# genjax-dev/genjax

Measured on AMD Instinct MI355X. Metric: particles/sec (particle-steps/s), bootstrap SMC sweep, linear-Gaussian SSM T=100, higher is better.
Workload: dtype f32; 1 GPU; BASELINE config 2: linear-Gaussian state-space (T=100), bootstrap SMC, systematic resampling every step; particles_per_gpu=1000000, particles_total=1000000, T=100, resampler=systematic, graph=True, key=314159

## Files before the change

genjax_amd/csrc/gmx_block.h:

```cpp
#pragma once
#define GMX_CHAIN_PRIO 2
#define GMX_SETPRIO __builtin_amdgcn_s_setprio(GMX_CHAIN_PRIO);
#include "gmx_math.h"
#define GMX_RTC_TILE 1024
#define GMX_RTC_MAX_TILES 2048
#if !defined(__HIPCC_RTC__)
#include "gmx_sizes.h"
static_assert(GMX_TILE == GMX_RTC_TILE && GMX_MAX_TILES == GMX_RTC_MAX_TILES, "gmx_block.h restates gmx_sizes.h for hiprtc");
#else
#define GMX_TILE GMX_RTC_TILE
#define GMX_MAX_TILES GMX_RTC_MAX_TILES
#endif

#define GMX_BLOCK 256
#define GMX_WAVE 64

template <int CTRL, int ROWMASK>
__device__ __forceinline__ uint32_t gmx_dpp(uint32_t identity, uint32_t v) {
  return (uint32_t)__builtin_amdgcn_update_dpp((int)identity, (int)v, CTRL, ROWMASK, 0xf, false);
}
#define GMX_DPP_SCAN_STEPS(STEP) \
  STEP(0x111, 0xf) STEP(0x112, 0xf) STEP(0x114, 0xf) STEP(0x118, 0xf) STEP(0x142, 0xa) STEP(0x143, 0xc)

#define GMX_DPP_ASM_ENTER "s_nop 4\n\t"
#define GMX_DPP_ASM_STEPS(OP) \
  OP("row_shr:1 row_mask:0xf bank_mask:0xf") OP("row_shr:2 row_mask:0xf bank_mask:0xf") \
  OP("row_shr:4 row_mask:0xf bank_mask:0xf") OP("row_shr:8 row_mask:0xf bank_mask:0xf") \
  OP("row_bcast:15 row_mask:0xa bank_mask:0xf") OP("row_bcast:31 row_mask:0xc bank_mask:0xf")

__device__ __forceinline__ float wave_max_scan(float v) {
#define GMX_OP(CTRL) "s_nop 1\n\tv_max_f32_dpp %0, %0, %0 " CTRL "\n\t"
  asm(GMX_DPP_ASM_ENTER GMX_DPP_ASM_STEPS(GMX_OP) : "+v"(v));
#undef GMX_OP
  return v;
}
__device__ __forceinline__ float wave_max(float v) {
  return gmx_u2f((uint32_t)__builtin_amdgcn_readlane((int)gmx_f2u(wave_max_scan(v)), 63));
}
__device__ __forceinline__ float wave_sum(float v) {
#pragma unroll
  for (int m = 32; m >= 1; m >>= 1) v = v + __shfl_xor(v, m, GMX_WAVE);
  return v;
}
__device__ __forceinline__ float block_max(float v, float* lds4) {
  v = wave_max(v);
  int w = threadIdx.x >> 6;
  __syncthreads();
  if ((threadIdx.x & 63) == 0) lds4[w] = v;
  __syncthreads();
  float r = gmx_rmax(gmx_rmax(lds4[0], lds4[1]), gmx_rmax(lds4[2], lds4[3]));
  return r;
}
__device__ __forceinline__ float block_sum(float v, float* lds4) {
  v = wave_sum(v);
  int w = threadIdx.x >> 6;
  __syncthreads();
  if ((threadIdx.x & 63) == 0) lds4[w] = v;
  __syncthreads();
  float r = (lds4[0] + lds4[1]) + (lds4[2] + lds4[3]);
  return r;
}

__device__ __forceinline__ void gmx_red_max(float* red_out, float* lds4, uint32_t row, float x, bool active) {
  float m = block_max(active ? x : -gmx_inf(), lds4);
  if (threadIdx.x == 0 && red_out) red_out[row] = m;
}
__device__ __forceinline__ void gmx_red_lse(float* red_out, float* lds4, uint32_t row, uint32_t rows, float x,
                                            bool active) {
  float m = block_max(active ? x : -gmx_inf(), lds4);
  float e = active ? gmx_expf(x - m) : 0.0f;
  if (!(m > -gmx_inf())) e = 0.0f;
  float s = block_sum(e, lds4);
  if (threadIdx.x == 0 && red_out) {
    red_out[row] = m;
    red_out[(size_t)rows + row] = s;
  }
}

__device__ __forceinline__ uint64_t wave_scan_u64(uint64_t v) {
  uint32_t lo = (uint32_t)v, hi = (uint32_t)(v >> 32);
#define GMX_OP(CTRL) "s_nop 1\n\tv_add_co_u32_dpp %0, vcc, %0, %0 " CTRL "\n\tv_addc_co_u32_dpp %1, vcc, %1, %1, vcc " CTRL "\n\t"
  asm(GMX_DPP_ASM_ENTER GMX_DPP_ASM_STEPS(GMX_OP) : "+v"(lo), "+v"(hi) : : "vcc");
#undef GMX_OP
  return ((uint64_t)hi << 32) | lo;
}
__device__ __forceinline__ uint64_t wave_last_u64(uint64_t v) {
  uint32_t lo = (uint32_t)__builtin_amdgcn_readlane((int)(uint32_t)v, 63);
  uint32_t hi = (uint32_t)__builtin_amdgcn_readlane((int)(uint32_t)(v >> 32), 63);
  return ((uint64_t)hi << 32) | lo;
}
__device__ __forceinline__ uint64_t wave_sum_u64(uint64_t v) { return wave_last_u64(wave_scan_u64(v)); }
__device__ __forceinline__ uint32_t wave_shr1_u32(uint32_t v, uint32_t first) { return gmx_dpp<0x138, 0xf>(first, v); }
__device__ __forceinline__ uint64_t shfl_up_u64(uint64_t v, int d) {
  uint32_t lo = (uint32_t)v, hi = (uint32_t)(v >> 32);
  lo = __shfl_up(lo, d, GMX_WAVE);
  hi = __shfl_up(hi, d, GMX_WAVE);
  return ((uint64_t)hi << 32) | lo;
}

__device__ __forceinline__ uint64_t weight_fixed(float lw, float ref, float scale) {
  return gmx_exp_fixed(lw - ref, (int)(gmx_f2u(scale) >> 23) - 127);
}

#define GMX_TP_MAX_TILES GMX_MAX_TILES
#define GMX_TP_PER_MAX (GMX_TP_MAX_TILES / GMX_BLOCK)
__device__ __forceinline__ void gmx_tile_prefix_block(const float* tmax, const uint64_t* agg, int n_tiles,
                                                      uint64_t* pref, float* lds4, uint64_t* lds8) {
  const int tid = (int)threadIdx.x, lane = tid & 63, wave = tid >> 6;
  const int per = (n_tiles + GMX_BLOCK - 1) / GMX_BLOCK;
  uint64_t ta[GMX_TP_PER_MAX];
  float tm[GMX_TP_PER_MAX];
#pragma unroll
  for (int r = 0; r < GMX_TP_PER_MAX; ++r) {
    ta[r] = 0ull; tm[r] = -gmx_inf();
    if (r < per) {
      const int t = tid * per + r;
      const int tc = t < n_tiles ? t : n_tiles - 1;
      ta[r] = agg[tc];
      tm[r] = tmax[tc];
    }
  }
  float M = -gmx_inf();
#pragma unroll
  for (int r = 0; r < GMX_TP_PER_MAX; ++r) {
    if (r < per) {
      const bool ok = tid * per + r < n_tiles;
      ta[r] = ok ? ta[r] : 0ull;
      tm[r] = ok ? tm[r] : -gmx_inf();
      M = gmx_rmax(M, tm[r]);
    }
  }
  M = block_max(M, lds4);
  const int32_t K = gmx_tile_exp(M);
  uint64_t P[GMX_TP_PER_MAX];
  uint64_t run = 0;
#pragma unroll
  for (int r = 0; r < GMX_TP_PER_MAX; ++r) {
    P[r] = run;
    if (r < per) run += gmx_tile_scale(ta[r], gmx_tile_exp(tm[r]), K);
  }
  const uint64_t inc = wave_scan_u64(run);
  __syncthreads();
  if (lane == 63) lds8[wave] = inc;
  __syncthreads();
  uint64_t wave_off = 0, total = 0;
#pragma unroll
  for (int w = 0; w < 4; ++w) { const uint64_t v = lds8[w]; total += v; wave_off += (w < wave) ? v : 0ull; }
  const uint64_t base = wave_off + (inc - run);
#pragma unroll
  for (int r = 0; r < GMX_TP_PER_MAX; ++r) {
    if (r < per) {
      const int t = tid * per + r;
      if (t < n_tiles) pref[t] = base + P[r];
    }
  }
  if (tid == 0) {
    pref[n_tiles] = total;
    pref[n_tiles + 1] = (uint64_t)gmx_f2u(M) | ((uint64_t)(uint32_t)K << 32);
  }
}
```

genjax_amd/csrc/gmx_kernels.hip:

```cpp
#include <hip/hip_runtime.h>
#include <hip/hiprtc.h>
#include <stdio.h>
#include <stdlib.h>
#include <string.h>
#include <sys/stat.h>
#include <unistd.h>

#include <new>
#include <atomic>
#include <string>
#include <vector>

#include "gmx_block.h"
#include "gmx_vm.h"
#include "gmx_resample.h"
#include "gmx_peer.h"
#include "gmx_sorted.h"
#include "gmx_offspring.h"
#include "gmx_shard_fill.h"

#define GMX_HIP(call)                                                        \
  do {                                                                       \
    hipError_t _e = (call);                                                  \
    if (_e != hipSuccess) return gmx_fail("%s (hip error %lld)", hipGetErrorString(_e), (long long)_e); \
// ... 309 lines not shown
extern "C" int gmx_program_despecialize(gmx_program* p, const char* why) {
  if (!p) return gmx_fail("gmx_program_despecialize: null program%s");
  if (!p->jit_fn) return 0;
  (void)hipDeviceSynchronize();
  (void)hipModuleUnload(p->jit_module);
  p->jit_fn = nullptr; p->jit_module = nullptr; p->jit_code_hash = 0;
  ++g_jit_rejected;
  (void)gmx_fail("specialised kernel rejected, the interpreter takes over: %s", why ? why : "");
  return 0;
}
extern "C" uint64_t gmx_program_code_hash(const gmx_program* p) { return p && p->jit_fn ? p->jit_code_hash : 0ull; }
extern "C" int gmx_program_writes_tile_stats(const gmx_program* p) {
  return p && p->jit_fn && p->jit_pp == 4 && p->n_redmax == 1 && !p->uses_lse ? 1 : 0;
}

extern "C" int gmx_program_set_fuse_resample(gmx_program* p) {
  if (!p) return gmx_fail("gmx_program_set_fuse_resample: null program%s");
  if (p->jit_fn) return gmx_fail("gmx_program_set_fuse_resample: the program is already specialised%s");
  p->fuse_rs = true;
  return 0;
}
extern "C" int gmx_program_set_fuse_resample_loop(gmx_program* p) {
  if (!p) return gmx_fail("gmx_program_set_fuse_resample_loop: null program%s");
  if (p->jit_fn) return gmx_fail("gmx_program_set_fuse_resample_loop: the program is already specialised%s");
  p->fuse_rs = true;
  p->fuse_rs_loop = true;
  return 0;
}
static int64_t rs_loop_grid(const gmx_program* p, int64_t tiles) {
  int64_t g = p->jit_resident_blocks > 0 ? p->jit_resident_blocks : 256;
  if (g > 1024) g = 1024;

  return tiles < g ? tiles : g;
}
extern "C" int gmx_program_fuses_resample(const gmx_program* p) {
  return p && p->jit_fn && p->fuse_rs && p->jit_pp == 4 && p->uses_gather && p->jit_gathers_pre ? 1 : 0;
}
extern "C" int gmx_program_set_fuse_shard_step(gmx_program* p) {
  if (!p) return gmx_fail("gmx_program_set_fuse_shard_step: null program%s");
  if (p->jit_fn) return gmx_fail("gmx_program_set_fuse_shard_step: the program is already specialised%s");
  p->fuse_sh = true;
  return 0;
}
extern "C" int gmx_program_fuses_shard_step(const gmx_program* p) {
  return p && p->jit_fn && p->fuse_sh && p->jit_pp == 4 && p->uses_gather && p->jit_gathers_pre ? 1 : 0;
}
extern "C" int64_t gmx_program_resident_particles(const gmx_program* p) {
  if (!p || !p->jit_fn) return 0;
  if (p->fuse_rs_loop && p->jit_pp == 4 && p->jit_resident_blocks > 0)
    return rs_loop_grid(p, 1024) * 16 * (int64_t)GMX_BLOCK * 4;
  return p->jit_resident_blocks * (int64_t)GMX_BLOCK * (int64_t)p->jit_pp;
}

extern "C" int gmx_program_set_background(gmx_program* p, uint32_t lds_pad) {
  if (!p) return gmx_fail("gmx_program_set_background: null program%s");
  if (p->jit_fn) return gmx_fail("gmx_program_set_background: the program is already specialised%s");
  if (lds_pad > 160u * 1024u) return gmx_fail("gmx_program_set_background: lds_pad above the 160 KB of a CU%s");
  p->background = true;
  p->lds_pad = lds_pad;
  return 0;
}

static uint64_t fnv1a(uint64_t h, const char* s, size_t n) {
  for (size_t i = 0; i < n; ++i) { h ^= (unsigned char)s[i]; h *= 0x100000001b3ull; }
  return h;
}

static std::string jit_cache_dir() {
  const char* e = getenv("GENMI_JIT_CACHE");
  if (e && e[0] == '0' && e[1] == '\0') return "";
  if (e && e[0]) return e;
  const char* x = getenv("XDG_CACHE_HOME");
  if (x && x[0]) return std::string(x) + "/genjax_amd/jit";
  const char* h = getenv("HOME");
  if (h && h[0]) return std::string(h) + "/.cache/genjax_amd/jit";
  return "";
}

static void mkdirs(const std::string& d) {
  for (size_t i = 1; i <= d.size(); ++i)
    if (i == d.size() || d[i] == '/') (void)mkdir(d.substr(0, i).c_str(), 0755);
}

static std::string jit_cache_path(const std::string& src) {
  std::string dir = jit_cache_dir();
  if (dir.empty()) return "";
  uint64_t h = fnv1a(0xcbf29ce484222325ull, src.data(), src.size());
  for (int k = 0; k < GMX_EMBED_COUNT; ++k) h = fnv1a(h, gmx_embed_src[k], strlen(gmx_embed_src[k]));
  int major = 0, minor = 0;
  (void)hiprtcVersion(&major, &minor);
  char buf[64];
  snprintf(buf, sizeof(buf), "/%016llx_rtc%d.%d_abi%d_e2.co", (unsigned long long)h, major, minor, GMX_ABI_VERSION);
  return dir + buf;
}

static const char* jit_opt_level() {
  const char* e = getenv("GENMI_JIT_OPT");
  return (e && (!strcmp(e, "-O1") || !strcmp(e, "-O2") || !strcmp(e, "-O0"))) ? e : "-O3";
}

static bool jit_cache_read(const std::string& path, std::vector<char>& code) {
  if (strcmp(jit_opt_level(), "-O3") != 0) return false;
  if (path.empty()) return false;
  FILE* f = fopen(path.c_str(), "rb");
  if (!f) return false;
  bool ok = false;
  if (fseek(f, 0, SEEK_END) == 0) {
    long n = ftell(f);
    if (n > 0 && n < (64l << 20) && fseek(f, 0, SEEK_SET) == 0) {
      code.resize((size_t)n);
      ok = fread(code.data(), 1, (size_t)n, f) == (size_t)n;
    }
  }
  fclose(f);
  return ok;
}

static bool jit_under_profiler() {
  const char* e = getenv("ROCP_TOOL_LIBRARIES");
  if (e && e[0]) return true;
  e = getenv("LD_PRELOAD");
  return e && strstr(e, "rocprofiler") != nullptr;
}

static void jit_cache_write(const std::string& path, const std::vector<char>& code) {
  if (path.empty() || jit_under_profiler() || strcmp(jit_opt_level(), "-O3") != 0) return;
  if (const char* f_ = getenv("GENMI_JIT_FAULT")) { if (f_[0] == '1') return; }
  mkdirs(path.substr(0, path.rfind('/')));
  char tmp[32];
  snprintf(tmp, sizeof(tmp), ".tmp%ld", (long)getpid());
  std::string t = path + tmp;
  FILE* f = fopen(t.c_str(), "wb");
  if (!f) return;
  bool ok = fwrite(code.data(), 1, code.size(), f) == code.size();
  ok = (fclose(f) == 0) && ok;
  if (!ok || rename(t.c_str(), path.c_str()) != 0) (void)remove(t.c_str());
}

static int jit_compile(const std::string& src, std::vector<char>& code) {
  hiprtcProgram prog;
  const char* hdr_src[GMX_EMBED_COUNT];
  const char* hdr_name[GMX_EMBED_COUNT];
  for (int k = 0; k < GMX_EMBED_COUNT; ++k) { hdr_src[k] = gmx_embed_src[k]; hdr_name[k] = gmx_embed_name[k]; }
  hiprtcResult rc = hiprtcCreateProgram(&prog, src.c_str(), "gmx_jit_program.hip", GMX_EMBED_COUNT, hdr_src, hdr_name);
  if (rc != HIPRTC_SUCCESS) return gmx_fail("hiprtcCreateProgram: %s", hiprtcGetErrorString(rc));
  const char* opts[4] = {"--offload-arch=gfx950", jit_opt_level(), "-std=c++17", "-ffp-contract=off"};
  rc = hiprtcCompileProgram(prog, 4, opts);
  if (rc != HIPRTC_SUCCESS) {
    size_t ls = 0;
    hiprtcGetProgramLogSize(prog, &ls);
    std::string log(ls + 1, '\0');
    if (ls) hiprtcGetProgramLog(prog, &log[0]);
    hiprtcDestroyProgram(&prog);
    if (log.size() > 400) log.resize(400);
    return gmx_fail("hiprtcCompileProgram failed: %s", log.c_str());
  }
  size_t cs = 0;
  hiprtcGetCodeSize(prog, &cs);
  code.resize(cs);
  hiprtcGetCode(prog, code.data());
  hiprtcDestroyProgram(&prog);
  return 0;
}

static int jit_load(gmx_program* p, const std::vector<char>& code) {
  hipModule_t mod;
  GMX_HIP(hipModuleLoadData(&mod, code.data()));
  hipFunction_t fn;
  hipError_t e = hipModuleGetFunction(&fn, mod, p->background ? "gmx_jit_background_kernel" : "gmx_jit_kernel");
  if (e != hipSuccess) { (void)hipModuleUnload(mod); return gmx_fail("hipModuleGetFunction: %s", hipGetErrorString(e)); }
  p->jit_module = mod;
  p->jit_fn = fn;
  p->jit_pp = jit_pp_for(p);
  p->jit_code_hash = fnv1a(0xcbf29ce484222325ull, code.data(), code.size());
  if (p->lds_pad > 48 * 1024) {
    hipError_t ea = hipFuncSetAttribute((const void*)fn, hipFuncAttributeMaxDynamicSharedMemorySize, (int)p->lds_pad);
    if (ea != hipSuccess) { (void)hipGetLastError(); p->lds_pad = 48 * 1024; }
  }
  p->jit_resident_blocks = 0;
  int per_cu = 0, dev = 0, cus = 0;
  if (hipModuleOccupancyMaxActiveBlocksPerMultiprocessor(&per_cu, fn, GMX_BLOCK, (size_t)p->lds_pad) == hipSuccess &&
      hipGetDevice(&dev) == hipSuccess &&
      hipDeviceGetAttribute(&cus, hipDeviceAttributeMultiprocessorCount, dev) == hipSuccess)
    p->jit_resident_blocks = (int64_t)per_cu * (int64_t)cus;
  else
    (void)hipGetLastError();
  return 0;
}

extern "C" int gmx_program_specialize(gmx_program* p) {
  if (!p) return gmx_fail("gmx_program_specialize: null program%s");
  if (p->jit_fn) return 0;
  if (!jit_enabled()) return gmx_fail("gmx_program_specialize: disabled by GENMI_JIT=0%s");
  if (p->n_instr == 0 || p->n_instr > 8192) return gmx_fail("gmx_program_specialize: program size out of range%s");
  const std::string src = jit_source(p, &p->jit_gathers_pre);
  const std::string path = jit_cache_path(src);
  std::vector<char> code;
  if (jit_cache_read(path, code)) {
    if (jit_load(p, code) == 0) return 0;
    (void)hipGetLastError();
  }
  if (jit_compile(src, code)) return 1;
  if (jit_load(p, code)) return 1;
  jit_cache_write(path, code);
  return 0;
}

extern "C" size_t gmx_specialize_dryrun2(const uint32_t* blob, size_t n_words, int flags, char* log_out, size_t log_cap,
                                         char* code_out, size_t code_cap);
extern "C" size_t gmx_specialize_dryrun(const uint32_t* blob, size_t n_words, char* log_out, size_t log_cap,
                                        char* code_out, size_t code_cap) {
  return gmx_specialize_dryrun2(blob, n_words, 0, log_out, log_cap, code_out, code_cap);
}
extern "C" size_t gmx_specialize_dryrun2(const uint32_t* blob, size_t n_words, int flags, char* log_out, size_t log_cap,
                                         char* code_out, size_t code_cap) {
  gmx_program P;
  if (parse_program(blob, n_words, P)) { if (log_out && log_cap) snprintf(log_out, log_cap, "%s", gmx_err_); return 0; }
  P.fuse_rs = (flags & 1) != 0 || (flags & 8) != 0;
  P.fuse_rs_loop = (flags & 8) != 0;
  P.background = (flags & 2) != 0;
  P.fuse_sh = (flags & 4) != 0;
  const gmx_program* p = &P;
  std::string src = jit_source(p);
  hiprtcProgram prog;
  const char* hdr_src[GMX_EMBED_COUNT];
  const char* hdr_name[GMX_EMBED_COUNT];
  for (int k = 0; k < GMX_EMBED_COUNT; ++k) { hdr_src[k] = gmx_embed_src[k]; hdr_name[k] = gmx_embed_name[k]; }
  if (hiprtcCreateProgram(&prog, src.c_str(), "gmx_jit_program.hip", GMX_EMBED_COUNT, hdr_src, hdr_name) != HIPRTC_SUCCESS)
    return 0;
  const char* opts[] = {"--offload-arch=gfx950", "-O3", "-std=c++17", "-ffp-contract=off"};
  hiprtcResult rc = hiprtcCompileProgram(prog, 4, opts);
  size_t ls = 0;
  hiprtcGetProgramLogSize(prog, &ls);
  if (log_out && log_cap) {
    std::string log(ls + 1, '\0');
    if (ls) hiprtcGetProgramLog(prog, &log[0]);
    snprintf(log_out, log_cap, "%s", log.c_str());
  }
  size_t cs = 0;
  if (rc == HIPRTC_SUCCESS) {
    hiprtcGetCodeSize(prog, &cs);
    if (code_out && code_cap >= cs) hiprtcGetCode(prog, code_out);
  }
  hiprtcDestroyProgram(&prog);
  return cs;
}

extern "C" int64_t gmx_program_grid(const gmx_program* p, int64_t n) {
  int64_t per = GMX_BLOCK;
  if (p && p->jit_fn && !p->uses_lse) per = (int64_t)GMX_BLOCK * p->jit_pp;
  return (n + per - 1) / per;
}

static int peer_check(const char* who, const gmx_peer& P, int64_t n_per_rank);
extern "C" int gmx_program_run(const gmx_program* p, int64_t n, const gmx_run_args* args,
                               gmx_stream stream) {
  if (!p || !args) return gmx_fail("gmx_program_run: null argument%s");
  if (n < 0) return gmx_fail("gmx_program_run: negative n%s");
  if (n == 0) return 0;
  if (n > (int64_t)0x7fffffff * GMX_BLOCK) return gmx_fail("gmx_program_run: n too large%s");
  for (uint32_t s = 0; s < p->n_in; ++s)
    if (!args->in_d[s]) return gmx_fail("gmx_program_run: input slot %s%lld is null", "", s);
  for (uint32_t s = 0; s < p->n_out; ++s)
    if (!args->out_d[s]) return gmx_fail("gmx_program_run: output slot %s%lld is null", "", s);
  for (uint32_t s = 0; s < p->n_tab; ++s)
    if (!args->tab_d[s]) return gmx_fail("gmx_program_run: table slot %s%lld is null", "", s);
  if (p->uses_gather && !args->ancestors_d)
    return gmx_fail("gmx_program_run: program gathers but ancestors_d is null%s");
  const bool fused_rs = args->rs.lw_d != nullptr;
  if (fused_rs) {
    const gmx_resample_in& q = args->rs;
    if (!gmx_program_fuses_resample(p))
      return gmx_fail("gmx_program_run: rs is set but this program cannot resample in its own launch "
                      "(gmx_program_set_fuse_resample before specialising; 4 particles per thread; gathering)%s");
    if (!q.tile_max_d || !q.tile_agg_d || !q.max_out_d || !q.total_out_d || !q.status_d)
      return gmx_fail("gmx_program_run: rs has a null pointer%s");
    if ((uintptr_t)q.lw_d & 15) return gmx_fail("gmx_program_run: rs.lw_d must be 16-byte aligned%s");
    if ((!p->fuse_rs_loop && (n + RS_TILE - 1) / RS_TILE > 1024) || n > gmx_program_resident_particles(p) ||
        n > (int64_t)GMX_ANC_INDEX_MASK + 1)
      return gmx_fail("gmx_program_run: rs: every workgroup of the launch must be resident at once (n <= 2^20 and "
                      "n <= gmx_program_resident_particles(); a looped program — gmx_program_set_fuse_resample_loop — "
                      "walks up to 16 tiles per workgroup: n <= 2^24)%s");
    if (q.shift < 1 || q.shift > 62) return gmx_fail("gmx_program_run: rs.shift out of range%s");
    int need = 0;
    while (((int64_t)1 << need) < n) ++need;
    if (q.shift + need > 62) return gmx_fail("gmx_program_run: rs.shift too large for n (overflow)%s");
    if (q.tag < 1u || q.tag > GMX_ANC_TAG_MAX) return gmx_fail("gmx_program_run: rs.tag must be in [1, 255]%s");
    if (args->tile_agg_d == q.tile_agg_d || (const float*)args->red_out_d == q.tile_max_d)
      return gmx_fail("gmx_program_run: rs reads the tile statistics this launch writes (use two sets)%s");
    for (uint32_t s = 0; s < p->n_out; ++s)
      if ((const void*)args->out_d[s] == (const void*)q.lw_d)
        return gmx_fail("gmx_program_run: rs.lw_d is also an output of this launch (use two buffers)%s");
  }
  const bool fused_sh = args->sh.lw_d != nullptr;
  if (fused_sh) {
    const gmx_shard_in& q = args->sh;
    if (fused_rs) return gmx_fail("gmx_program_run: rs and sh are both set%s");
    if (!gmx_program_fuses_shard_step(p))
      return gmx_fail("gmx_program_run: sh is set but this program cannot route a sharded step in its own launch "
                      "(gmx_program_set_fuse_shard_step before specialising; 4 particles per thread; gathering)%s");
    if (!q.stats_own_d || !q.plan_d || !q.total_out_d || !q.max_out_d || !q.status_d)
      return gmx_fail("gmx_program_run: sh has a null pointer%s");
    if (((uintptr_t)q.lw_d & 15) || ((uintptr_t)q.stats_own_d & 7))
      return gmx_fail("gmx_program_run: sh.lw_d must be 16-byte and sh.stats_own_d 8-byte aligned%s");
    if (peer_check("gmx_program_run (sh)", q.peer, n)) return 1;
    if (q.peer.world > 8 || (int64_t)q.peer.world * q.peer.tiles > 4 * GMX_BLOCK)
      return gmx_fail("gmx_program_run: sh: world <= 8 and world * tiles <= 1024%s");
    if (n + (int64_t)q.peer.world * q.peer.capacity > (int64_t)GMX_ANC_INDEX_MASK + 1)
      return gmx_fail("gmx_program_run: sh: n + world * capacity must fit the 21-bit index of an ancestor word%s");
    if (n > gmx_program_resident_particles(p))
      return gmx_fail("gmx_program_run: sh: every workgroup of the launch must be resident at once "
                      "(n <= gmx_program_resident_particles())%s");
    if (q.shift < 1 || q.shift > 62) return gmx_fail("gmx_program_run: sh.shift out of range%s");
    if (q.tag < 1u || q.tag > GMX_ANC_TAG_MAX) return gmx_fail("gmx_program_run: sh.tag must be in [1, 255]%s");
// ... 2842 lines not shown
```

genjax_amd/csrc/gmx_offspring.h:

```cpp
#pragma once
#include "gmx_block.h"
#include "gmx_resample.h"
#include "gmx_sorted.h"

#define CDF_VEC_OT 4
#ifndef RS_THREADS
#define RS_THREADS 256
#endif
#define RS_TILE (RS_THREADS * CDF_VEC_OT)
#define RS_MAX_TILES GMX_MAX_TILES
static_assert(RS_TILE == GMX_TILE && RS_THREADS == GMX_BLOCK, "resampling tiles are the CDF's definition tiles");
static_assert(RS_MAX_TILES % GMX_BLOCK == 0, "tile table shape");

#define GMX_ANC_TAG_SHIFT 24
#define GMX_ANC_INDEX_MASK 0xffffffu
#define GMX_ANC_TAG_MAX 255u
__device__ __forceinline__ void gmx_store_u32x4_sc1(uint32_t* p, uint32_t a, uint32_t b, uint32_t c, uint32_t d) {
  typedef uint32_t v4 __attribute__((ext_vector_type(4)));
  v4 v; v.x = a; v.y = b; v.z = c; v.w = d;
  asm volatile("s_nop 1\n\tglobal_store_dwordx4 %0, %1, off sc1\n\ts_nop 1" :: "v"(p), "v"(v) : "memory");
}
__device__ __forceinline__ void gmx_store_u32_sc1(uint32_t* p, uint32_t a) {
  __hip_atomic_store(p, a, __ATOMIC_RELAXED, __HIP_MEMORY_SCOPE_AGENT);
}

typedef uint32_t rs_u32x4_a4 __attribute__((ext_vector_type(4), aligned(4)));
typedef uint32_t sorted_u32x2_a4 __attribute__((ext_vector_type(2), aligned(4)));
struct sorted_ctx {
  const uint32_t* slow; const uint32_t* guide; const uint64_t* toff;
  uint64_t stot, gmax; uint32_t sh, mask; double ratio;
};
__device__ __forceinline__ sorted_ctx sorted_ctx_of(const uint32_t* table, int64_t n, uint64_t total, uint64_t stot, uint32_t sh) {
  const gmx_sorted_layout L = gmx_sorted_layout_of(n);
  sorted_ctx X;
  X.slow = table; X.guide = table + L.off_guide;
  X.toff = reinterpret_cast<const uint64_t*>(table + L.off_toff);
  X.stot = stot;
  X.sh = sh;
  X.mask = (1u << X.sh) - 1u;
  X.gmax = X.stot >> X.sh;
  X.ratio = (double)X.stot / (double)(total ? total : 1ull);
  return X;
}
__device__ __forceinline__ int64_t sorted_below_exact(const sorted_ctx& X, uint64_t c, uint64_t total, int64_t j, int64_t n) {
  const u128 R = mul64(c, X.stot);
  j = j < 0 ? 0 : (j > n ? n : j);
  auto below = [&](int64_t k) {
    const uint64_t off = X.toff[k >> 10];
    const uint64_t S = off + (uint64_t)(uint32_t)(X.slow[k] - (uint32_t)off);
    return gt128(R, mul64(S, total));
  };
  while (j > 0 && !below(j - 1)) --j;
  while (j < n && below(j)) ++j;
  return j;
}

#define RS_TPB 1
#define GMX_KEEP_BRANCH asm volatile("")
#define RS_BLOCK (GMX_BLOCK * RS_TPB)
#define RS_WAVES (RS_BLOCK / GMX_WAVE)
static_assert(RS_MAX_TILES % RS_BLOCK == 0, "tile table shape");
#define RS_FILL_SLOTS 2048
template <int kind, int PER, bool TAGGED>
__device__ __forceinline__ void
gmx_offspring_tile_body(uint32_t k0, uint32_t k1, uint32_t u0_host, const float* __restrict__ lw,
                        const float* __restrict__ tmax, const uint64_t* __restrict__ agg, int64_t n, int n_tiles, float scale,
                        float* __restrict__ max_out, uint64_t* __restrict__ total_out, int32_t* __restrict__ anc,
                        const uint32_t* __restrict__ uslot, uint32_t tag,
                        int tile0 = -1, uint64_t a_prefix = 0ull, uint64_t a_total = 0ull, uint64_t a_mk = 0ull) {
  const int blk = tile0 >= 0 ? tile0 : (int)blockIdx.x;
  const uint32_t tagw = TAGGED ? (tag << GMX_ANC_TAG_SHIFT) : 0u;
  __shared__ uint64_t s_below[RS_WAVES], s_all[RS_WAVES], s_scan[RS_WAVES], s_g[RS_TPB];
  __shared__ float s_max[RS_WAVES];
  const int lane = threadIdx.x & 63, wave = threadIdx.x >> 6;
  const int grp = RS_TPB > 1 ? (int)(threadIdx.x >> 8) : 0, ltid = threadIdx.x & (GMX_BLOCK - 1);
  const int first_tile = blk * RS_TPB;
  const int my_tile = first_tile + grp;
  const bool tile_ok = my_tile < n_tiles;
  const int tile_c = tile_ok ? my_tile : n_tiles - 1;
  const int64_t i0 = (int64_t)tile_c * RS_TILE + (int64_t)ltid * CDF_VEC_OT;
  float x[CDF_VEC_OT];
  const bool full_tile = (int64_t)(tile_c + 1) * RS_TILE <= n;
  if (full_tile) {
    float4 v = *reinterpret_cast<const float4*>(lw + i0);
    x[0] = v.x; x[1] = v.y; x[2] = v.z; x[3] = v.w;
  } else {
#pragma unroll
    for (int c = 0; c < CDF_VEC_OT; ++c) {
      const int64_t ic = i0 + c < n ? i0 + c : n - 1;
      const float xv = lw[ic];
      x[c] = (i0 + c < n) ? xv : -gmx_inf();
    }
  }
  constexpr bool PREF = (PER == 0);
  constexpr int PERN = PREF ? 1 : PER;
  static_assert(PER >= 0 && PER * RS_BLOCK <= RS_MAX_TILES, "rows of the tile table per thread");
  static_assert(!PREF || RS_TPB == 1, "the prefix form works on one tile per block");
  uint64_t ta[PERN];
  float tm[PERN];
  uint64_t pf_prefix = 0, pf_total = 0, pf_mk = 0;
  if (PREF) {
    if (agg) { pf_prefix = agg[tile_c]; pf_total = agg[n_tiles]; pf_mk = agg[n_tiles + 1]; }
    else { pf_prefix = a_prefix; pf_total = a_total; pf_mk = a_mk; }
  } else {
#pragma unroll
    for (int r = 0; r < PERN; ++r) {
      ta[r] = 0ull; tm[r] = -gmx_inf();
      if (r * RS_BLOCK < n_tiles) {
        const int t = r * RS_BLOCK + (int)threadIdx.x;
        const int tc = t < n_tiles ? t : n_tiles - 1;
        ta[r] = agg[tc];
        tm[r] = tmax[tc];
      }
    }
  }
  const float tmax_mine = tmax[tile_c];
  uint64_t sx_stot = 0; uint32_t sx_sh = 0;
  if constexpr (kind == GMX_RESAMPLE_MULTINOMIAL_SORTED) {
    const gmx_sorted_layout L = gmx_sorted_layout_of(n);
    sx_stot = reinterpret_cast<const uint64_t*>(uslot + L.off_toff)[L.tiles];
    sx_sh = uslot[L.off_sh];
  }
  __builtin_amdgcn_sched_barrier(0);
  if (!PREF) {
#pragma unroll
    for (int r = 0; r < PERN; ++r) {
      if (r * RS_BLOCK < n_tiles && (r + 1) * RS_BLOCK > n_tiles) {
        GMX_KEEP_BRANCH;
        const int t = r * RS_BLOCK + (int)threadIdx.x;
        ta[r] = (t < n_tiles) ? ta[r] : 0ull;
        tm[r] = (t < n_tiles) ? tm[r] : -gmx_inf();
      }
    }
  }
  const int32_t k_b = gmx_tile_exp(tmax_mine);
  const float ref_b = gmx_tile_ref(k_b);
  float M = -gmx_inf();
  if (PREF) {
    M = gmx_u2f((uint32_t)pf_mk);
  } else {
#pragma unroll
    for (int r = 0; r < PERN; ++r)
      if (r * RS_BLOCK < n_tiles) M = gmx_rmax(M, tm[r]);
    M = wave_max(M);
  }
  uint64_t q[CDF_VEC_OT];
  uint64_t run = 0;
#pragma unroll
  for (int c = 0; c < CDF_VEC_OT; ++c) q[c] = weight_fixed(x[c], ref_b, scale);
  if (!(tile_ok && full_tile)) {
    GMX_KEEP_BRANCH;
#pragma unroll
    for (int c = 0; c < CDF_VEC_OT; ++c) q[c] = (tile_ok && i0 + c < n) ? q[c] : 0ull;
  }
#pragma unroll
  for (int c = 0; c < CDF_VEC_OT; ++c) {
    run += q[c];
    q[c] = run;
  }
  const uint64_t inc = wave_scan_u64(run);
  if (!PREF && lane == 0) s_max[wave] = M;
  if (lane == 63) s_scan[wave] = inc;
  __syncthreads();
  if (!PREF) {
    M = s_max[0];
#pragma unroll
    for (int w = 1; w < RS_WAVES; ++w) M = gmx_rmax(M, s_max[w]);
  }
  uint64_t wave_off = 0;
#pragma unroll
  for (int w = 0; w < 4; ++w) wave_off += (w < (wave & 3)) ? s_scan[4 * grp + w] : 0ull;
  const uint64_t loc = wave_off + (inc - run);
  const int32_t K = PREF ? (int32_t)(uint32_t)(pf_mk >> 32) : gmx_tile_exp(M);
  uint64_t prefix = 0, total = 0;
  if (PREF) {
    prefix = pf_prefix; total = pf_total;
  } else {
    uint64_t below = 0, all = 0;
#pragma unroll
    for (int r = 0; r < PERN; ++r) {
      if (r * RS_BLOCK < n_tiles) {
        const int t = r * RS_BLOCK + (int)threadIdx.x;
        const uint64_t G = gmx_tile_scale(ta[r], gmx_tile_exp(tm[r]), K);
        all += G;
        if ((r + 1) * RS_BLOCK <= first_tile) { GMX_KEEP_BRANCH; below += G; }
        else if (r * RS_BLOCK < first_tile) { GMX_KEEP_BRANCH; below += (t < first_tile) ? G : 0ull; }
        if constexpr (RS_TPB > 1)
          if (t >= first_tile && t < first_tile + RS_TPB) s_g[t - first_tile] = G;
      }
    }
    below = wave_sum_u64(below);
    all = wave_sum_u64(all);
    if (lane == 0) { s_below[wave] = below; s_all[wave] = all; }
    __syncthreads();
#pragma unroll
    for (int w = 0; w < RS_WAVES; ++w) { prefix += s_below[w]; total += s_all[w]; }
    if constexpr (RS_TPB > 1) {
#pragma unroll
      for (int j = 0; j < RS_TPB; ++j) prefix += (j < grp) ? s_g[j] : 0ull;
    }
  }
  if (blk == 0 && threadIdx.x == 0) { *total_out = total; *max_out = M; }
  if (!tile_ok) return;
  gmx_key key; key.k0 = k0; key.k1 = k1;
  if (total == 0) {
#pragma unroll
    for (int c = 0; c < CDF_VEC_OT; ++c)
      if (i0 + c < n) {
        if (TAGGED) gmx_store_u32_sc1(reinterpret_cast<uint32_t*>(anc) + (i0 + c), (uint32_t)(n - 1) | tagw);
        else anc[i0 + c] = (int32_t)(n - 1);
      }
    return;
  }
  const double n_over_total = (double)n / (double)total;
  const double eps = (double)n * 0x1p-44 + 0x1p-40;
  const int32_t n32 = (int32_t)n;
  uint64_t cv[CDF_VEC_OT + 1];
  cv[0] = prefix + gmx_tile_scale(loc, k_b, K);
#pragma unroll
  for (int c = 0; c < CDF_VEC_OT; ++c) cv[c + 1] = prefix + gmx_tile_scale(loc + q[c], k_b, K);
  if (!full_tile) {
    GMX_KEEP_BRANCH;
#pragma unroll
    for (int c = 0; c < CDF_VEC_OT; ++c) cv[c + 1] = (i0 + c < n) ? cv[c + 1] : total;
  }
  int32_t e[CDF_VEC_OT + 1];
  bool near = false;
  uint32_t near_bits = 0;
  constexpr bool SORTED = (kind == GMX_RESAMPLE_MULTINOMIAL_SORTED);
  sorted_ctx SX;
  if constexpr (SORTED) SX = sorted_ctx_of(uslot, n, total, sx_stot, sx_sh);
  auto below_est = [&](uint64_t c) -> sb_est {
    return slots_below_est<kind == GMX_RESAMPLE_MULTINOMIAL_SORTED ? GMX_RESAMPLE_SYSTEMATIC : kind>(
        key, u0_host, c, total, n_over_total, eps, n32, uslot);
  };
  sb_est R[CDF_VEC_OT + 1];
  if constexpr (SORTED) {
    uint32_t mv[CDF_VEC_OT + 1], gv[CDF_VEC_OT + 1], lov[CDF_VEC_OT + 1], hiv[CDF_VEC_OT + 1], kv[CDF_VEC_OT + 1];
    auto eval = [&](const int c0, const int c1) {
#pragma unroll
      for (int c = c0; c <= c1; ++c) {
        const double cd = __builtin_fma((double)(uint32_t)(cv[c] >> 32), 4294967296.0, (double)(uint32_t)cv[c]);
        const double t = cd * SX.ratio;
        const uint64_t tq = (uint64_t)t;
        const double frac = t - (double)tq;
        const double teps = __builtin_fma(t, 0x1p-49, 0x1p-40);
        R[c].near = (frac < teps) || (frac > 1.0 - teps);
        const uint64_t gq = tq >> SX.sh;
        gv[c] = (uint32_t)(gq < SX.gmax ? gq : SX.gmax);
        mv[c] = (uint32_t)tq & SX.mask;
      }
#pragma unroll
      for (int c = c0; c <= c1; ++c) {
        const sorted_u32x2_a4 gh = *reinterpret_cast<const sorted_u32x2_a4*>(SX.guide + gv[c]);
        lov[c] = gh.x; hiv[c] = gh.y;
      }
#pragma unroll
      for (int c = c0; c <= c1; ++c) {
        hiv[c] = hiv[c] < (uint32_t)n32 ? hiv[c] : (uint32_t)n32;
        lov[c] = lov[c] < hiv[c] ? lov[c] : hiv[c];
      }
      rs_u32x4_a4 pa[CDF_VEC_OT + 1], pb[CDF_VEC_OT + 1];
#pragma unroll
      for (int c = c0; c <= c1; ++c) {
        pa[c] = *reinterpret_cast<const rs_u32x4_a4*>(SX.slow + lov[c]);
        pb[c] = *reinterpret_cast<const rs_u32x4_a4*>(SX.slow + lov[c] + 4u);
      }
      bool more = false;
#pragma unroll
      for (int c = c0; c <= c1; ++c) {
        const uint32_t pv[8] = {pa[c].x, pa[c].y, pa[c].z, pa[c].w, pb[c].x, pb[c].y, pb[c].z, pb[c].w};
        uint32_t k = lov[c];
#pragma unroll
        for (uint32_t i = 0; i < 8u; ++i) k += (lov[c] + i < hiv[c] && (pv[i] & SX.mask) <= mv[c]) ? 1u : 0u;
        kv[c] = k;
        more |= (k == lov[c] + 8u && k < hiv[c]);
      }
      if (more) {
#pragma unroll 1
        for (int c = c0; c <= c1; ++c) {
          uint32_t k = kv[c];
          if (k == lov[c] + 8u)
            while (k < hiv[c] && (SX.slow[k] & SX.mask) <= mv[c]) ++k;
          kv[c] = k;
        }
      }
#pragma unroll
      for (int c = c0; c <= c1; ++c) {
        R[c].j = (int32_t)kv[c];
        if (cv[c] == 0ull) { R[c].j = 0; R[c].near = false; }
        if (cv[c] >= total) { R[c].j = n32; R[c].near = false; }
      }
    };
    R[0].j = 0; R[0].near = false;
    eval(1, CDF_VEC_OT);
    if (wave == 0) eval(0, 0);
  } else {
#pragma unroll
    for (int c = 1; c <= CDF_VEC_OT; ++c) R[c] = below_est(cv[c]);
    R[0].j = 0; R[0].near = false;
    if (__builtin_amdgcn_readfirstlane(wave) == 0) R[0] = below_est(cv[0]);
  }
#pragma unroll
  for (int c = 1; c <= CDF_VEC_OT; ++c) {
    e[c] = R[c].j;
    near_bits |= R[c].near ? (1u << c) : 0u;
  }
  {
    const sb_est r = R[0];
    near_bits |= (lane == 0 && r.near) ? 1u : 0u;
    e[0] = (int32_t)wave_shr1_u32((uint32_t)e[CDF_VEC_OT], (uint32_t)r.j);
    if (lane == 0) e[0] = r.j;
  }
  near = near_bits != 0u;
  if (__any(near)) {
    const uint64_t D = (uint64_t)n << 23;
    int32_t fixed0 = e[0];
#pragma unroll 1
    for (int c = 0; c <= CDF_VEC_OT; ++c) {
      if (near_bits & (1u << c)) {
        const uint64_t cc = c == 0 ? cv[0] : c == 1 ? cv[1] : c == 2 ? cv[2] : c == 3 ? cv[3] : cv[4];
        const int32_t j0 = c == 0 ? e[0] : c == 1 ? e[1] : c == 2 ? e[2] : c == 3 ? e[3] : e[4];
        int32_t j;
        if constexpr (SORTED) j = (int32_t)sorted_below_exact(SX, cc, total, (int64_t)j0, n);
        else j = (int32_t)slots_below_exact(kind, key, (uint64_t)u0_host, cc, D, total, (int64_t)j0, n);
        if (c == 0) fixed0 = j; else if (c == 1) e[1] = j; else if (c == 2) e[2] = j; else if (c == 3) e[3] = j; else e[4] = j;
      }
    }
    const uint32_t up = wave_shr1_u32((uint32_t)e[CDF_VEC_OT], (uint32_t)fixed0);
    e[0] = (lane == 0) ? fixed0 : (int32_t)up;
  }
  __shared__ int32_t s_edge[RS_WAVES];
  if (lane == 63) s_edge[wave] = e[CDF_VEC_OT];
  const int32_t e4 = e[4];
  const int32_t src0 = (int32_t)i0;
  static_assert(RS_TPB == 1, "the LDS fill works on one tile per block");
  __shared__ __attribute__((aligned(16))) uint32_t s_mark[RS_FILL_SLOTS];
  __shared__ int32_t s_rng[2];
  __shared__ uint32_t s_carry[RS_WAVES];
  if (threadIdx.x == 0) s_rng[0] = e[0];
  if (threadIdx.x == RS_BLOCK - 1) s_rng[1] = e4;
  reinterpret_cast<uint4*>(s_mark)[threadIdx.x] = make_uint4(0u, 0u, 0u, 0u);
  reinterpret_cast<uint4*>(s_mark)[threadIdx.x + RS_BLOCK] = make_uint4(0u, 0u, 0u, 0u);
  __syncthreads();
  if (lane == 0 && wave > 0) e[0] = s_edge[wave - 1];
  const int32_t T0 = __builtin_amdgcn_readfirstlane(s_rng[0]), T1 = __builtin_amdgcn_readfirstlane(s_rng[1]);
  for (int32_t base = T0; base < T1; base += RS_FILL_SLOTS) {
    if (base != T0) {
      reinterpret_cast<uint4*>(s_mark)[threadIdx.x] = make_uint4(0u, 0u, 0u, 0u);
      reinterpret_cast<uint4*>(s_mark)[threadIdx.x + RS_BLOCK] = make_uint4(0u, 0u, 0u, 0u);
      __syncthreads();
    }
#pragma unroll
    for (int c = 0; c < CDF_VEC_OT; ++c) {
      const int32_t lo = e[c] > base ? e[c] : base;
      if (e[c + 1] > lo && lo - base < RS_FILL_SLOTS) s_mark[lo - base] = (uint32_t)(src0 + c);
    }
    __syncthreads();
    uint4 a = reinterpret_cast<const uint4*>(s_mark)[2 * threadIdx.x];
    uint4 b = reinterpret_cast<const uint4*>(s_mark)[2 * threadIdx.x + 1];
    a.y = a.y > a.x ? a.y : a.x; a.z = a.z > a.y ? a.z : a.y; a.w = a.w > a.z ? a.w : a.z;
    b.x = b.x > a.w ? b.x : a.w; b.y = b.y > b.x ? b.y : b.x; b.z = b.z > b.y ? b.z : b.y; b.w = b.w > b.z ? b.w : b.z;
    const uint32_t incl = gmx_wave_umax_scan(b.w);
    uint32_t carry = wave_shr1_u32(incl, 0u);
    if (lane == 63) s_carry[wave] = incl;
    __syncthreads();
#pragma unroll
    for (int w = 0; w < RS_WAVES - 1; ++w) { const uint32_t v = s_carry[w]; carry = (w < wave && v > carry) ? v : carry; }
    a.x = a.x > carry ? a.x : carry; a.y = a.y > carry ? a.y : carry; a.z = a.z > carry ? a.z : carry; a.w = a.w > carry ? a.w : carry;
    b.x = b.x > carry ? b.x : carry; b.y = b.y > carry ? b.y : carry; b.z = b.z > carry ? b.z : carry; b.w = b.w > carry ? b.w : carry;
    const int32_t j = base + 8 * (int32_t)threadIdx.x;
    if (j + 8 <= T1) {
      rs_u32x4_a4 va, vb;
      va.x = a.x; va.y = a.y; va.z = a.z; va.w = a.w; vb.x = b.x; vb.y = b.y; vb.z = b.z; vb.w = b.w;
      if (TAGGED) {
        gmx_store_u32x4_sc1(reinterpret_cast<uint32_t*>(anc) + j, va.x | tagw, va.y | tagw, va.z | tagw, va.w | tagw);
        gmx_store_u32x4_sc1(reinterpret_cast<uint32_t*>(anc) + j + 4, vb.x | tagw, vb.y | tagw, vb.z | tagw, vb.w | tagw);
      } else {
        *reinterpret_cast<rs_u32x4_a4*>(anc + j) = va;
        *reinterpret_cast<rs_u32x4_a4*>(anc + j + 4) = vb;
      }
    } else {
      if (j + 0 < T1) { if (TAGGED) gmx_store_u32_sc1(reinterpret_cast<uint32_t*>(anc) + j + 0, a.x | tagw); else anc[j + 0] = (int32_t)a.x; }
      if (j + 1 < T1) { if (TAGGED) gmx_store_u32_sc1(reinterpret_cast<uint32_t*>(anc) + j + 1, a.y | tagw); else anc[j + 1] = (int32_t)a.y; }
      if (j + 2 < T1) { if (TAGGED) gmx_store_u32_sc1(reinterpret_cast<uint32_t*>(anc) + j + 2, a.z | tagw); else anc[j + 2] = (int32_t)a.z; }
      if (j + 3 < T1) { if (TAGGED) gmx_store_u32_sc1(reinterpret_cast<uint32_t*>(anc) + j + 3, a.w | tagw); else anc[j + 3] = (int32_t)a.w; }
      if (j + 4 < T1) { if (TAGGED) gmx_store_u32_sc1(reinterpret_cast<uint32_t*>(anc) + j + 4, b.x | tagw); else anc[j + 4] = (int32_t)b.x; }
      if (j + 5 < T1) { if (TAGGED) gmx_store_u32_sc1(reinterpret_cast<uint32_t*>(anc) + j + 5, b.y | tagw); else anc[j + 5] = (int32_t)b.y; }
      if (j + 6 < T1) { if (TAGGED) gmx_store_u32_sc1(reinterpret_cast<uint32_t*>(anc) + j + 6, b.z | tagw); else anc[j + 6] = (int32_t)b.z; }
      if (j + 7 < T1) { if (TAGGED) gmx_store_u32_sc1(reinterpret_cast<uint32_t*>(anc) + j + 7, b.w | tagw); else anc[j + 7] = (int32_t)b.w; }
    }
  }
}



__device__ __forceinline__ void
gmx_tile_table_pass(const float* __restrict__ tmax, const uint64_t* __restrict__ agg, int n_tiles, int blk, int G, int C,
                    uint64_t* __restrict__ s_pf , uint64_t& total, uint64_t& mk) {
  __shared__ float s_tm[RS_WAVES];
  __shared__ uint64_t s_acc[RS_WAVES][2];
  const int lane = threadIdx.x & 63, wave = threadIdx.x >> 6;
  float M = -gmx_inf();
  for (int t = (int)threadIdx.x; t < n_tiles; t += RS_BLOCK) M = gmx_rmax(M, tmax[t]);
  M = wave_max(M);
  if (lane == 0) s_tm[wave] = M;
  __syncthreads();
  M = s_tm[0];
#pragma unroll
  for (int w = 1; w < RS_WAVES; ++w) M = gmx_rmax(M, s_tm[w]);
  const int32_t K = gmx_tile_exp(M);
  uint64_t running = 0;
#pragma clang loop unroll(disable)
  for (int c = 0; c < C; ++c) {
    const int lo = c * G, hi = (lo + G < n_tiles) ? lo + G : n_tiles, mine = lo + blk;
    uint64_t tot = 0, part = 0;
    for (int tb = lo; tb < hi; tb += RS_BLOCK) {
      const int t = tb + (int)threadIdx.x;
      if (t < hi) {
        const uint64_t g_ = gmx_tile_scale(agg[t], gmx_tile_exp(tmax[t]), K);
        tot += g_;
        if (tb + RS_BLOCK <= mine) { GMX_KEEP_BRANCH; part += g_; }
        else if (tb < mine) { GMX_KEEP_BRANCH; part += (t < mine) ? g_ : 0ull; }
      }
    }
    tot = wave_sum_u64(tot);
    part = wave_sum_u64(part);
    if (lane == 0) { s_acc[wave][0] = tot; s_acc[wave][1] = part; }
    __syncthreads();
    uint64_t T_ = 0, P_ = 0;
#pragma unroll
    for (int w = 0; w < RS_WAVES; ++w) { T_ += s_acc[w][0]; P_ += s_acc[w][1]; }
    if (threadIdx.x == 0) s_pf[c] = running + P_;
    running += T_;
    __syncthreads();
  }
  total = running;
  mk = (uint64_t)gmx_f2u(M) | ((uint64_t)(uint32_t)K << 32);
}
```

Before: 73.92 billion particle-steps/s.

## Fuse paired wave u64 sums, widen tagged stores, add JIT option hashing

```diff
diff --git a/genjax_amd/csrc/gmx_block.h b/genjax_amd/csrc/gmx_block.h
--- a/genjax_amd/csrc/gmx_block.h
+++ b/genjax_amd/csrc/gmx_block.h
@@ -27,6 +27,10 @@
   OP("row_shr:1 row_mask:0xf bank_mask:0xf") OP("row_shr:2 row_mask:0xf bank_mask:0xf") \
   OP("row_shr:4 row_mask:0xf bank_mask:0xf") OP("row_shr:8 row_mask:0xf bank_mask:0xf") \
   OP("row_bcast:15 row_mask:0xa bank_mask:0xf") OP("row_bcast:31 row_mask:0xc bank_mask:0xf")
+#define GMX_DPP_ASM_HALF_STEPS(OP) \
+  OP("row_shr:1 row_mask:0xf bank_mask:0xf") OP("row_shr:2 row_mask:0xf bank_mask:0xf") \
+  OP("row_shr:4 row_mask:0xf bank_mask:0xf") OP("row_shr:8 row_mask:0xf bank_mask:0xf") \
+  OP("row_bcast:15 row_mask:0xa bank_mask:0xf")
 
 __device__ __forceinline__ float wave_max_scan(float v) {
 #define GMX_OP(CTRL) "s_nop 1\n\tv_max_f32_dpp %0, %0, %0 " CTRL "\n\t"
@@ -90,6 +94,17 @@
   return ((uint64_t)hi << 32) | lo;
 }
 __device__ __forceinline__ uint64_t wave_sum_u64(uint64_t v) { return wave_last_u64(wave_scan_u64(v)); }
+__device__ __forceinline__ void wave_sum2_u64(uint64_t& a, uint64_t& b) {
+  const auto slo = __builtin_amdgcn_permlane32_swap((uint32_t)a, (uint32_t)b, false, false);
+  const auto shi = __builtin_amdgcn_permlane32_swap((uint32_t)(a >> 32), (uint32_t)(b >> 32), false, false);
+  const uint64_t v = (((uint64_t)(uint32_t)shi[0] << 32) | (uint32_t)slo[0]) + (((uint64_t)(uint32_t)shi[1] << 32) | (uint32_t)slo[1]);
+  uint32_t lo = (uint32_t)v, hi = (uint32_t)(v >> 32);
+#define GMX_OP(CTRL) "s_nop 1\n\tv_add_co_u32_dpp %0, vcc, %0, %0 " CTRL "\n\tv_addc_co_u32_dpp %1, vcc, %1, %1, vcc " CTRL "\n\t"
+  asm(GMX_DPP_ASM_ENTER GMX_DPP_ASM_HALF_STEPS(GMX_OP) : "+v"(lo), "+v"(hi) : : "vcc");
+#undef GMX_OP
+  a = ((uint64_t)(uint32_t)__builtin_amdgcn_readlane((int)hi, 31) << 32) | (uint32_t)__builtin_amdgcn_readlane((int)lo, 31);
+  b = ((uint64_t)(uint32_t)__builtin_amdgcn_readlane((int)hi, 63) << 32) | (uint32_t)__builtin_amdgcn_readlane((int)lo, 63);
+}
 __device__ __forceinline__ uint32_t wave_shr1_u32(uint32_t v, uint32_t first) { return gmx_dpp<0x138, 0xf>(first, v); }
 __device__ __forceinline__ uint64_t shfl_up_u64(uint64_t v, int d) {
   uint32_t lo = (uint32_t)v, hi = (uint32_t)(v >> 32);
diff --git a/genjax_amd/csrc/gmx_kernels.hip b/genjax_amd/csrc/gmx_kernels.hip
--- a/genjax_amd/csrc/gmx_kernels.hip
+++ b/genjax_amd/csrc/gmx_kernels.hip
@@ -415,10 +415,26 @@
     if (i == d.size() || d[i] == '/') (void)mkdir(d.substr(0, i).c_str(), 0755);
 }
 
-static std::string jit_cache_path(const std::string& src) {
+struct jit_options {
+  const char* v[5];
+  int n;
+  std::string text() const {
+    std::string s;
+    for (int k = 0; k < n; ++k) { s += v[k]; s += ' '; }
+    return s;
+  }
+};
+static jit_options jit_options_of(bool background, const char* level) {
+  jit_options o = {{"--offload-arch=gfx950", level, "-std=c++17", "-ffp-contract=off", nullptr}, 4};
+  if (!background) o.v[o.n++] = "-fno-slp-vectorize";
+  return o;
+}
+
+static std::string jit_cache_path(const std::string& src, const std::string& opts) {
   std::string dir = jit_cache_dir();
   if (dir.empty()) return "";
   uint64_t h = fnv1a(0xcbf29ce484222325ull, src.data(), src.size());
+  h = fnv1a(h, opts.data(), opts.size());
   for (int k = 0; k < GMX_EMBED_COUNT; ++k) h = fnv1a(h, gmx_embed_src[k], strlen(gmx_embed_src[k]));
   int major = 0, minor = 0;
   (void)hiprtcVersion(&major, &minor);
@@ -470,15 +486,14 @@
   if (!ok || rename(t.c_str(), path.c_str()) != 0) (void)remove(t.c_str());
 }
 
-static int jit_compile(const std::string& src, std::vector<char>& code) {
+static int jit_compile(const std::string& src, const jit_options& opts, std::vector<char>& code) {
   hiprtcProgram prog;
   const char* hdr_src[GMX_EMBED_COUNT];
   const char* hdr_name[GMX_EMBED_COUNT];
   for (int k = 0; k < GMX_EMBED_COUNT; ++k) { hdr_src[k] = gmx_embed_src[k]; hdr_name[k] = gmx_embed_name[k]; }
   hiprtcResult rc = hiprtcCreateProgram(&prog, src.c_str(), "gmx_jit_program.hip", GMX_EMBED_COUNT, hdr_src, hdr_name);
   if (rc != HIPRTC_SUCCESS) return gmx_fail("hiprtcCreateProgram: %s", hiprtcGetErrorString(rc));
-  const char* opts[4] = {"--offload-arch=gfx950", jit_opt_level(), "-std=c++17", "-ffp-contract=off"};
-  rc = hiprtcCompileProgram(prog, 4, opts);
+  rc = hiprtcCompileProgram(prog, opts.n, const_cast<const char**>(opts.v));
   if (rc != HIPRTC_SUCCESS) {
     size_t ls = 0;
     hiprtcGetProgramLogSize(prog, &ls);
@@ -527,16 +542,28 @@
   if (!jit_enabled()) return gmx_fail("gmx_program_specialize: disabled by GENMI_JIT=0%s");
   if (p->n_instr == 0 || p->n_instr > 8192) return gmx_fail("gmx_program_specialize: program size out of range%s");
   const std::string src = jit_source(p, &p->jit_gathers_pre);
-  const std::string path = jit_cache_path(src);
+  const jit_options opts = jit_options_of(p->background, jit_opt_level());
+  const std::string path = jit_cache_path(src, opts.text());
   std::vector<char> code;
   if (jit_cache_read(path, code)) {
     if (jit_load(p, code) == 0) return 0;
     (void)hipGetLastError();
   }
-  if (jit_compile(src, code)) return 1;
+  if (jit_compile(src, opts, code)) return 1;
   if (jit_load(p, code)) return 1;
   jit_cache_write(path, code);
   return 0;
+}
+
+extern "C" size_t gmx_jit_cache_path_of(const char* src, const char* opts, char* out, size_t cap) {
+  const std::string path = jit_cache_path(src ? src : "", opts ? opts : "");
+  if (out && cap) snprintf(out, cap, "%s", path.c_str());
+  return path.size();
+}
+extern "C" size_t gmx_jit_options_of(int flags, char* out, size_t cap) {
+  const std::string t = jit_options_of((flags & 2) != 0, "-O3").text();
+  if (out && cap) snprintf(out, cap, "%s", t.c_str());
+  return t.size();
 }
 
 extern "C" size_t gmx_specialize_dryrun2(const uint32_t* blob, size_t n_words, int flags, char* log_out, size_t log_cap,
@@ -561,8 +588,8 @@
   for (int k = 0; k < GMX_EMBED_COUNT; ++k) { hdr_src[k] = gmx_embed_src[k]; hdr_name[k] = gmx_embed_name[k]; }
   if (hiprtcCreateProgram(&prog, src.c_str(), "gmx_jit_program.hip", GMX_EMBED_COUNT, hdr_src, hdr_name) != HIPRTC_SUCCESS)
     return 0;
-  const char* opts[] = {"--offload-arch=gfx950", "-O3", "-std=c++17", "-ffp-contract=off"};
-  hiprtcResult rc = hiprtcCompileProgram(prog, 4, opts);
+  const jit_options opts = jit_options_of(P.background, "-O3");
+  hiprtcResult rc = hiprtcCompileProgram(prog, opts.n, const_cast<const char**>(opts.v));
   size_t ls = 0;
   hiprtcGetProgramLogSize(prog, &ls);
   if (log_out && log_cap) {
diff --git a/genjax_amd/csrc/gmx_offspring.h b/genjax_amd/csrc/gmx_offspring.h
--- a/genjax_amd/csrc/gmx_offspring.h
+++ b/genjax_amd/csrc/gmx_offspring.h
@@ -19,6 +19,12 @@
   typedef uint32_t v4 __attribute__((ext_vector_type(4)));
   v4 v; v.x = a; v.y = b; v.z = c; v.w = d;
   asm volatile("s_nop 1\n\tglobal_store_dwordx4 %0, %1, off sc1\n\ts_nop 1" :: "v"(p), "v"(v) : "memory");
+}
+__device__ __forceinline__ void gmx_store_u32x8_sc1(uint32_t* base_uniform, uint32_t off, uint4 a, uint4 b) {
+  typedef uint32_t v4 __attribute__((ext_vector_type(4)));
+  v4 va, vb; va.x = a.x; va.y = a.y; va.z = a.z; va.w = a.w; vb.x = b.x; vb.y = b.y; vb.z = b.z; vb.w = b.w;
+  asm volatile("s_nop 1\n\tglobal_store_dwordx4 %0, %1, %3 sc1\n\tglobal_store_dwordx4 %0, %2, %3 offset:16 sc1\n\ts_nop 1"
+               :: "v"(off), "v"(va), "v"(vb), "s"(base_uniform) : "memory");
 }
 __device__ __forceinline__ void gmx_store_u32_sc1(uint32_t* p, uint32_t a) {
   __hip_atomic_store(p, a, __ATOMIC_RELAXED, __HIP_MEMORY_SCOPE_AGENT);
@@ -57,6 +63,7 @@
 
 #define RS_TPB 1
 #define GMX_KEEP_BRANCH asm volatile("")
+__device__ __forceinline__ uint64_t rs_zext_here(uint32_t o) { asm volatile("" : "+v"(o)); return (uint64_t)o; }
 #define RS_BLOCK (GMX_BLOCK * RS_TPB)
 #define RS_WAVES (RS_BLOCK / GMX_WAVE)
 static_assert(RS_MAX_TILES % RS_BLOCK == 0, "tile table shape");
@@ -98,6 +105,7 @@
   static_assert(!PREF || RS_TPB == 1, "the prefix form works on one tile per block");
   uint64_t ta[PERN];
   float tm[PERN];
+  const uint32_t tid4 = threadIdx.x * 4u;
   uint64_t pf_prefix = 0, pf_total = 0, pf_mk = 0;
   if (PREF) {
     if (agg) { pf_prefix = agg[tile_c]; pf_total = agg[n_tiles]; pf_mk = agg[n_tiles + 1]; }
@@ -107,10 +115,18 @@
     for (int r = 0; r < PERN; ++r) {
       ta[r] = 0ull; tm[r] = -gmx_inf();
       if (r * RS_BLOCK < n_tiles) {
-        const int t = r * RS_BLOCK + (int)threadIdx.x;
-        const int tc = t < n_tiles ? t : n_tiles - 1;
-        ta[r] = agg[tc];
-        tm[r] = tmax[tc];
+        if ((r + 1) * RS_BLOCK <= n_tiles) {
+          GMX_KEEP_BRANCH;
+          uint32_t r0 = (uint32_t)(r * RS_BLOCK);
+          asm volatile("" : "+s"(r0));
+          ta[r] = *reinterpret_cast<const uint64_t*>(reinterpret_cast<const char*>(agg + r0) + rs_zext_here(tid4 * 2u));
+          tm[r] = *reinterpret_cast<const float*>(reinterpret_cast<const char*>(tmax + r0) + rs_zext_here(tid4));
+        } else {
+          const int t = r * RS_BLOCK + (int)threadIdx.x;
+          const int tc = t < n_tiles ? t : n_tiles - 1;
+          ta[r] = agg[tc];
+          tm[r] = tmax[tc];
+        }
       }
     }
   }
@@ -189,8 +205,7 @@
           if (t >= first_tile && t < first_tile + RS_TPB) s_g[t - first_tile] = G;
       }
     }
-    below = wave_sum_u64(below);
-    all = wave_sum_u64(all);
+    wave_sum2_u64(below, all);
     if (lane == 0) { s_below[wave] = below; s_all[wave] = all; }
     __syncthreads();
 #pragma unroll
@@ -333,7 +348,7 @@
   __shared__ int32_t s_edge[RS_WAVES];
   if (lane == 63) s_edge[wave] = e[CDF_VEC_OT];
   const int32_t e4 = e[4];
-  const int32_t src0 = (int32_t)i0;
+  const uint32_t src0t = (uint32_t)(int32_t)i0 | tagw;
   static_assert(RS_TPB == 1, "the LDS fill works on one tile per block");
   __shared__ __attribute__((aligned(16))) uint32_t s_mark[RS_FILL_SLOTS];
   __shared__ int32_t s_rng[2];
@@ -354,7 +369,7 @@
 #pragma unroll
     for (int c = 0; c < CDF_VEC_OT; ++c) {
       const int32_t lo = e[c] > base ? e[c] : base;
-      if (e[c + 1] > lo && lo - base < RS_FILL_SLOTS) s_mark[lo - base] = (uint32_t)(src0 + c);
+      if (e[c + 1] > lo && lo - base < RS_FILL_SLOTS) s_mark[lo - base] = src0t + (uint32_t)c;
     }
     __syncthreads();
     uint4 a = reinterpret_cast<const uint4*>(s_mark)[2 * threadIdx.x];
@@ -374,21 +389,20 @@
       rs_u32x4_a4 va, vb;
       va.x = a.x; va.y = a.y; va.z = a.z; va.w = a.w; vb.x = b.x; vb.y = b.y; vb.z = b.z; vb.w = b.w;
       if (TAGGED) {
-        gmx_store_u32x4_sc1(reinterpret_cast<uint32_t*>(anc) + j, va.x | tagw, va.y | tagw, va.z | tagw, va.w | tagw);
-        gmx_store_u32x4_sc1(reinterpret_cast<uint32_t*>(anc) + j + 4, vb.x | tagw, vb.y | tagw, vb.z | tagw, vb.w | tagw);
+        gmx_store_u32x8_sc1(reinterpret_cast<uint32_t*>(anc) + base, 32u * threadIdx.x, a, b);
       } else {
         *reinterpret_cast<rs_u32x4_a4*>(anc + j) = va;
         *reinterpret_cast<rs_u32x4_a4*>(anc + j + 4) = vb;
       }
     } else {
-      if (j + 0 < T1) { if (TAGGED) gmx_store_u32_sc1(reinterpret_cast<uint32_t*>(anc) + j + 0, a.x | tagw); else anc[j + 0] = (int32_t)a.x; }
-      if (j + 1 < T1) { if (TAGGED) gmx_store_u32_sc1(reinterpret_cast<uint32_t*>(anc) + j + 1, a.y | tagw); else anc[j + 1] = (int32_t)a.y; }
-      if (j + 2 < T1) { if (TAGGED) gmx_store_u32_sc1(reinterpret_cast<uint32_t*>(anc) + j + 2, a.z | tagw); else anc[j + 2] = (int32_t)a.z; }
-      if (j + 3 < T1) { if (TAGGED) gmx_store_u32_sc1(reinterpret_cast<uint32_t*>(anc) + j + 3, a.w | tagw); else anc[j + 3] = (int32_t)a.w; }
-      if (j + 4 < T1) { if (TAGGED) gmx_store_u32_sc1(reinterpret_cast<uint32_t*>(anc) + j + 4, b.x | tagw); else anc[j + 4] = (int32_t)b.x; }
-      if (j + 5 < T1) { if (TAGGED) gmx_store_u32_sc1(reinterpret_cast<uint32_t*>(anc) + j + 5, b.y | tagw); else anc[j + 5] = (int32_t)b.y; }
-      if (j + 6 < T1) { if (TAGGED) gmx_store_u32_sc1(reinterpret_cast<uint32_t*>(anc) + j + 6, b.z | tagw); else anc[j + 6] = (int32_t)b.z; }
-      if (j + 7 < T1) { if (TAGGED) gmx_store_u32_sc1(reinterpret_cast<uint32_t*>(anc) + j + 7, b.w | tagw); else anc[j + 7] = (int32_t)b.w; }
+      if (j + 0 < T1) { if (TAGGED) gmx_store_u32_sc1(reinterpret_cast<uint32_t*>(anc) + j + 0, a.x); else anc[j + 0] = (int32_t)a.x; }
+      if (j + 1 < T1) { if (TAGGED) gmx_store_u32_sc1(reinterpret_cast<uint32_t*>(anc) + j + 1, a.y); else anc[j + 1] = (int32_t)a.y; }
+      if (j + 2 < T1) { if (TAGGED) gmx_store_u32_sc1(reinterpret_cast<uint32_t*>(anc) + j + 2, a.z); else anc[j + 2] = (int32_t)a.z; }
+      if (j + 3 < T1) { if (TAGGED) gmx_store_u32_sc1(reinterpret_cast<uint32_t*>(anc) + j + 3, a.w); else anc[j + 3] = (int32_t)a.w; }
+      if (j + 4 < T1) { if (TAGGED) gmx_store_u32_sc1(reinterpret_cast<uint32_t*>(anc) + j + 4, b.x); else anc[j + 4] = (int32_t)b.x; }
+      if (j + 5 < T1) { if (TAGGED) gmx_store_u32_sc1(reinterpret_cast<uint32_t*>(anc) + j + 5, b.y); else anc[j + 5] = (int32_t)b.y; }
+      if (j + 6 < T1) { if (TAGGED) gmx_store_u32_sc1(reinterpret_cast<uint32_t*>(anc) + j + 6, b.z); else anc[j + 6] = (int32_t)b.z; }
+      if (j + 7 < T1) { if (TAGGED) gmx_store_u32_sc1(reinterpret_cast<uint32_t*>(anc) + j + 7, b.w); else anc[j + 7] = (int32_t)b.w; }
     }
   }
 }
@@ -424,8 +438,7 @@
         else if (tb < mine) { GMX_KEEP_BRANCH; part += (t < mine) ? g_ : 0ull; }
       }
     }
-    tot = wave_sum_u64(tot);
-    part = wave_sum_u64(part);
+    wave_sum2_u64(tot, part);
     if (lane == 0) { s_acc[wave][0] = tot; s_acc[wave][1] = part; }
     __syncthreads();
     uint64_t T_ = 0, P_ = 0;
```

New measurement: 75.65 billion particle-steps/s, median of 6. 1.02x the previous value.
